# m4rch1n0/vqvae

Measured on AMD Instinct MI355X. Metric: latents/sec through geodesic kNN+APSP+K-medoids, higher is better.
Workload: dtype f64-exact(u32 fixed point)

## Files before the change

### include/geo_hip.h

```cpp
#ifndef GEO_HIP_H
#define GEO_HIP_H

#include <stddef.h>
#include <stdint.h>

#ifdef __cplusplus
extern "C" {
#endif

#define GEO_OK 0
#define GEO_E_ARG (-1)
#define GEO_E_WORKSPACE (-2)
#define GEO_E_HIP (-3)
#define GEO_E_NOCONV (-4)

int geo_version(void);
const char *geo_last_error(void);

int geo_set_option(const char *name, int32_t value);

size_t geo_sssp_workspace_bytes(int32_t n, int64_t nnz, int32_t n_sources);

int geo_sssp_multi(const int32_t *indptr, const int32_t *indices, const float *weights,
                   int32_t n, int64_t nnz, const int32_t *sources, int32_t n_sources,
// ... 129 lines not shown
                          const int32_t *src, const int32_t *dst, int64_t n_edges, int32_t batch_size,
                          float *len_out, void *ws, size_t ws_bytes, void *stream);
size_t geo_jvp_edges_part_workspace_bytes(const geo_decoder_desc *dec, int64_t n_nodes, int64_t n_edges, int64_t build_edges,
                                          int32_t batch_size);
int geo_decoder_jvp_edges_part(const geo_decoder_desc *dec, const float *z, int64_t n_nodes,
                               const int32_t *src, const int32_t *dst, int64_t n_edges, int64_t build_edges, int32_t batch_size,
                               float *len_out, void *ws, size_t ws_bytes, void *stream);

#define GEO_JVP_FRONT_VALU 0
#define GEO_JVP_FRONT_MFMA 1
#define GEO_JVP_MID_PIPE 0
#define GEO_JVP_MID_PIPE_DEDUP 1
#define GEO_JVP_MID_ALL 2
#define GEO_JVP_MID_ALL_TANGENT 3
#define GEO_JVP_MID_CHUNK 4
#define GEO_JVP_BACK_MFMA 0
#define GEO_JVP_BACK_PER_NODE 1
#define GEO_JVP_BACK_DEDUP 2
#define GEO_JVP_BACK_VALU 3
#define GEO_JVP_PLAN_FRONT(p) ((p) & 3)
#define GEO_JVP_PLAN_DMAX(p) (16 << (((p) >> 2) & 3))
#define GEO_JVP_PLAN_MID(p) (((p) >> 4) & 15)
#define GEO_JVP_PLAN_BACK(p) (((p) >> 8) & 15)
#define GEO_JVP_PER_NODE 0x1000
#define GEO_JVP_NODE_JACOBIAN 0x2000
#define GEO_JVP_DEDUP 0x4000
#define GEO_JVP_FRONT_ONCE 0x8000
#define GEO_JVP_PLAN_PASSES(p) ((p) >> 16)
int geo_jvp_plan(const geo_decoder_desc *dec, int64_t n_nodes, int64_t n_edges, int32_t batch_size, int32_t graph_edges,
                 size_t ws_bytes);
int geo_jvp_plan_part(const geo_decoder_desc *dec, int64_t n_nodes, int64_t n_edges, int64_t build_edges, int32_t batch_size,
                      int32_t graph_edges, size_t ws_bytes);
int geo_jvp_head_stream(const geo_decoder_desc *dec, int64_t n_nodes, int64_t n_edges, int32_t batch_size, int32_t graph_edges);

int geo_decoder_jvp_pairs(const geo_decoder_desc *dec, const float *z_start, const float *z_end,
                          int64_t n_edges, int32_t batch_size, float *len_out,
                          void *ws, size_t ws_bytes, void *stream);


typedef struct geo_vanilla_decoder_desc {
    int32_t latent_dim;
    int32_t c1, c2;
    int32_t out_channels;
    int32_t out_size;
    const float *At;
    const float *c;
    const float *w2p;
    const float *scale2;
    const float *shift2;
    const float *w3p;
    const float *b3;
} geo_vanilla_decoder_desc;

size_t geo_vanilla_jvp_workspace_bytes(const geo_vanilla_decoder_desc *dec, int64_t n_edges);
size_t geo_vanilla_jvp_edges_workspace_bytes(const geo_vanilla_decoder_desc *dec, int64_t n_nodes, int64_t n_edges);
int geo_vanilla_jvp_pairs(const geo_vanilla_decoder_desc *dec, const float *z_start, const float *z_end, int64_t n_edges,
                          int32_t batch_size, float *len_out, void *ws, size_t ws_bytes, void *stream);
int geo_vanilla_jvp_edges(const geo_vanilla_decoder_desc *dec, const float *z, int64_t n_nodes, const int32_t *src,
                          const int32_t *dst, int64_t n_edges, int32_t batch_size, float *len_out, void *ws, size_t ws_bytes,
                          void *stream);

size_t geo_vanilla_decode_workspace_bytes(const geo_vanilla_decoder_desc *dec, int64_t n);
int geo_vanilla_decode(const geo_vanilla_decoder_desc *dec, const float *z, const int32_t *index, int64_t n, float *logits_out,
                       void *ws, size_t ws_bytes, void *stream);

typedef struct geo_spatial_image_decoder_desc {
// ... 145 lines not shown
```

### vqvae_amd/_lib.py

```python
import ctypes
import os

import torch

_HERE = os.path.dirname(os.path.abspath(__file__))
LIB_PATH = os.path.join(_HERE, "libgeo_hip.so")

c_p = ctypes.c_void_p
i32, i64, sz = ctypes.c_int32, ctypes.c_int64, ctypes.c_size_t


class DecoderDesc(ctypes.Structure):
    _fields_ = ([(n, i32) for n in ("latent_dim", "c0", "c1", "c2", "out_channels", "out_size", "norm",
                                    "bn_train", "groups1", "groups2")]
                + [("eps", ctypes.c_float)]
                + [(n, c_p) for n in ("w_in", "b_in", "w1", "b1", "g1", "be1", "rm1", "rv1",
                                      "w2", "b2", "g2", "be2", "rm2", "rv2", "w3", "b3")]
                + [("update_running", i32), ("momentum", ctypes.c_float)])


class VanillaDecoderDesc(ctypes.Structure):
    _fields_ = ([(n, i32) for n in ("latent_dim", "c1", "c2", "out_channels", "out_size")]
                + [(n, c_p) for n in ("At", "c", "w2p", "scale2", "shift2", "w3p", "b3")])

# ... 45 lines not shown
    "geo_cell_costs_workspace_bytes": (sz, [i32, i64, i32, i32]),
    "geo_cell_costs_min_workspace_bytes": (sz, [i32, i64, i32, i32]),
    "geo_cell_costs": (ctypes.c_int, [c_p, c_p, c_p, i32, i64, c_p, c_p, c_p, i32, i32, i32, c_p, c_p, sz, c_p, c_p]),
    "geo_kpp_resident_max_nodes": (i32, []),
    "geo_kpp_chain": (ctypes.c_int, [c_p, c_p, c_p, i32, c_p, c_p, c_p, c_p, c_p, i32, i32, i32, i32, i32, c_p, sz, c_p, c_p]),
    "geo_knn_workspace_bytes": (sz, [i64, i32]),
    "geo_knn_topk": (ctypes.c_int, [c_p, i64, i32, i32, i32, i64, i64, c_p, c_p, c_p, sz, c_p]),
    "geo_knn_query_workspace_bytes": (sz, [i64, i64, i32]),
    "geo_knn_query_min_workspace_bytes": (sz, [i64, i32]),
    "geo_knn_query": (ctypes.c_int, [c_p, i64, c_p, i64, i32, i32, i32, c_p, c_p, c_p, sz, c_p]),
    "geo_knn_last_path": (ctypes.c_int, []),
    "geo_knn_thresholds": (ctypes.c_int, [c_p, i64, i32, i32, i32, i64, i64, i32, c_p, c_p, sz, c_p]),
    "geo_nearest_foreign_workspace_bytes": (sz, [i64, i32]),
    "geo_nearest_foreign": (ctypes.c_int, [c_p, i64, i32, i32, c_p, c_p, i64, c_p, c_p, c_p, sz, c_p]),
    "geo_bridge_components_workspace_bytes": (sz, [i64, i32, i32]),
    "geo_bridge_components": (ctypes.c_int, [c_p, i64, i32, i32, c_p, i32, c_p, c_p, c_p, c_p, sz, c_p]),
    "geo_csr_insert_workspace_bytes": (sz, [i32, i64]),
    "geo_csr_insert_count": (ctypes.c_int, [c_p, c_p, i32, c_p, c_p, c_p, i64, c_p, c_p, c_p, sz, c_p]),
    "geo_csr_insert_fill": (ctypes.c_int, [c_p, c_p, c_p, i32, i64, c_p, c_p, c_p, c_p, sz, c_p]),
    "geo_symmetrize_workspace_bytes": (sz, [i32, i32]),
    "geo_symmetrize_count": (ctypes.c_int, [c_p, c_p, i32, i32, i32, c_p, c_p, c_p, sz, c_p]),
    "geo_symmetrize_fill": (ctypes.c_int, [c_p, c_p, i32, i32, i32, c_p, c_p, c_p, c_p, sz, c_p]),
    "geo_upper_edges_count": (ctypes.c_int, [c_p, c_p, i32, c_p, c_p, c_p, sz, c_p]),
    "geo_upper_edges_fill": (ctypes.c_int, [c_p, c_p, i32, c_p, c_p, c_p, c_p, c_p]),
    "geo_cc_workspace_bytes": (sz, [i32]),
    "geo_connected_components": (ctypes.c_int, [c_p, c_p, i32, c_p, c_p, c_p, sz, c_p]),
    "geo_csr_compact_workspace_bytes": (sz, [i32]),
    "geo_csr_compact_count": (ctypes.c_int, [c_p, c_p, c_p, i32, c_p, i32, c_p, c_p, c_p, c_p, c_p, sz, c_p]),
    "geo_csr_compact_fill": (ctypes.c_int, [c_p, c_p, c_p, i32, c_p, i32, c_p, c_p, c_p, c_p, c_p]),
    "geo_jvp_workspace_bytes": (sz, [ctypes.POINTER(DecoderDesc), i64, i32]),
    "geo_jvp_edges_workspace_bytes": (sz, [ctypes.POINTER(DecoderDesc), i64, i64, i32]),
    "geo_jvp_plan": (ctypes.c_int, [ctypes.POINTER(DecoderDesc), i64, i64, i32, i32, sz]),
    "geo_jvp_head_stream": (ctypes.c_int, [ctypes.POINTER(DecoderDesc), i64, i64, i32, i32]),
    "geo_decoder_jvp_edges": (ctypes.c_int, [ctypes.POINTER(DecoderDesc), c_p, i64, c_p, c_p, i64, i32, c_p, c_p, sz, c_p]),
    "geo_jvp_edges_part_workspace_bytes": (sz, [ctypes.POINTER(DecoderDesc), i64, i64, i64, i32]),
    "geo_jvp_plan_part": (ctypes.c_int, [ctypes.POINTER(DecoderDesc), i64, i64, i64, i32, i32, sz]),
    "geo_decoder_jvp_edges_part": (ctypes.c_int, [ctypes.POINTER(DecoderDesc), c_p, i64, c_p, c_p, i64, i64, i32, c_p, c_p, sz,
                                                  c_p]),
    "geo_decoder_jvp_pairs": (ctypes.c_int, [ctypes.POINTER(DecoderDesc), c_p, c_p, i64, i32, c_p, c_p, sz, c_p]),
    "geo_vanilla_jvp_workspace_bytes": (sz, [ctypes.POINTER(VanillaDecoderDesc), i64]),
    "geo_vanilla_jvp_edges_workspace_bytes": (sz, [ctypes.POINTER(VanillaDecoderDesc), i64, i64]),
    "geo_vanilla_jvp_pairs": (ctypes.c_int, [ctypes.POINTER(VanillaDecoderDesc), c_p, c_p, i64, i32, c_p, c_p, sz, c_p]),
    "geo_vanilla_jvp_edges": (ctypes.c_int, [ctypes.POINTER(VanillaDecoderDesc), c_p, i64, c_p, c_p, i64, i32, c_p, c_p, sz, c_p]),
    "geo_vanilla_decode_workspace_bytes": (sz, [ctypes.POINTER(VanillaDecoderDesc), i64]),
    "geo_vanilla_decode": (ctypes.c_int, [ctypes.POINTER(VanillaDecoderDesc), c_p, c_p, i64, c_p, c_p, sz, c_p]),
    "geo_spatial_decode_workspace_bytes": (sz, [ctypes.POINTER(SpatialImageDecoderDesc), i64]),
    "geo_spatial_decode": (ctypes.c_int, [ctypes.POINTER(SpatialImageDecoderDesc), c_p, c_p, c_p, i64, c_p, c_p, sz, c_p]),
    "geo_image_encode_workspace_bytes": (sz, [ctypes.POINTER(ImageEncoderDesc), i64]),
    "geo_image_encode": (ctypes.c_int, [ctypes.POINTER(ImageEncoderDesc), c_p, i64, c_p, c_p, c_p, sz, c_p]),
    "geo_lpips_alex_workspace_bytes": (sz, [i64]),
    "geo_lpips_alex": (ctypes.c_int, [ctypes.POINTER(LPIPSAlexDesc), c_p, c_p, i64, c_p, c_p, c_p, sz, c_p]),
    "geo_gather_edge_weights":(ctypes.c_int, [c_p, c_p, i64, c_p, c_p]),
    "geo_prior_sample_workspace_bytes": (sz, [ctypes.POINTER(PriorDesc), i32, i32]),
    "geo_prior_sample": (ctypes.c_int, [ctypes.POINTER(PriorDesc), c_p, i32, i32, c_p, c_p, ctypes.c_float, i32, c_p, c_p, i32,
                                        c_p, sz, c_p]),
    "geo_kmeans_workspace_bytes": (sz, [i64, i32, i32, i32, i32]),
    "geo_kmeans_assign": (ctypes.c_int, [c_p, i64, i32, c_p, i32, c_p, c_p, c_p, c_p, sz, c_p]),
    "geo_kmeans_pp": (ctypes.c_int, [c_p, i64, i32, i32, i32, i32, c_p, c_p, c_p, c_p, c_p, sz, c_p]),
    "geo_kmeans_lloyd": (ctypes.c_int, [c_p, i64, i32, i32, i32, c_p, i32, ctypes.c_double, c_p, c_p, c_p, c_p, c_p, c_p, c_p,
                                        sz, c_p]),
    "geo_image_pair_moments": (ctypes.c_int, [c_p, c_p, i64, i64, c_p, c_p]),
    "geo_cluster_label_scores": (ctypes.c_int, [c_p, c_p, i64, i32, i32, i32, c_p, c_p, c_p, c_p, c_p, c_p]),
    "geo_feature_workspace_bytes": (sz, [i64, i32]),
    "geo_feature_colstats": (ctypes.c_int, [c_p, i64, i32, i64, c_p, c_p, c_p, c_p, sz, c_p]),
    "geo_feature_gram": (ctypes.c_int, [c_p, i64, i32, i64, c_p, c_p, c_p, c_p, sz, c_p]),
    "geo_feature_project": (ctypes.c_int, [c_p, i64, i32, i64, c_p, c_p, c_p, i32, c_p, c_p]),
# ... 57 lines not shown
```

### vqvae_amd/csrc/common.hip

```cpp
#include "geo_common.h"

#include <cstdlib>
#include <cstring>

namespace geo {

namespace {
struct OptionName { const char *name, *env; int Options::*field; };
const OptionName kOptionNames[] = {
    {"sssp_sb", "GEO_SSSP_SB", &Options::sssp_sb},
    {"sssp_act", "GEO_SSSP_ACT", &Options::sssp_act},
    {"sssp_sparse_div", "GEO_SSSP_SPARSE_DIV", &Options::sssp_sparse_div},
    {"sssp_map_div", "GEO_SSSP_MAP_DIV", &Options::sssp_map_div},
    {"sssp_group", "GEO_SSSP_GROUP", &Options::sssp_group},
    {"sssp_grouped_cap", "GEO_SSSP_GROUPED_CAP", &Options::sssp_grouped_cap},
    {"sssp_trace", "GEO_SSSP_TRACE", &Options::sssp_trace},
    {"sssp_u32", "GEO_SSSP_U32", &Options::sssp_u32},
    {"sssp_push", "GEO_SSSP_PUSH", &Options::sssp_push},
    {"sssp_order", "GEO_SSSP_ORDER", &Options::sssp_order},
    {"sssp_delta", "GEO_SSSP_DELTA", &Options::sssp_delta},
    {"sssp_push_blocks", "GEO_SSSP_PUSH_BLOCKS", &Options::sssp_push_blocks},
    {"knn_filter", "GEO_KNN_FILTER", &Options::knn_filter},
    {"kpp_grid", "GEO_KPP_GRID", &Options::kpp_grid},
    {"kpp_profile", "GEO_KPP_PROFILE", &Options::kpp_profile},
    {"jvp_mid", "GEO_JVP_MID", &Options::jvp_mid},
    {"jvp_back_valu", "GEO_JVP_BACK_VALU", &Options::jvp_back_valu},
    {"jvp_front_valu", "GEO_JVP_FRONT_VALU", &Options::jvp_front_valu},
    {"jvp_per_node", "GEO_JVP_PER_NODE", &Options::jvp_per_node},
    {"jvp_node_jacobian", "GEO_JVP_NODE_JACOBIAN", &Options::jvp_node_jacobian},
    {"jvp_start_dedup", "GEO_JVP_START_DEDUP", &Options::jvp_start_dedup},
    {"jvp_front_once", "GEO_JVP_FRONT_ONCE", &Options::jvp_front_once},
    {"jvp_head_stream", "GEO_JVP_HEAD_STREAM", &Options::jvp_head_stream},
};
Options from_environment() {
    Options o;
    for (const OptionName &e : kOptionNames) {
        const char *v = getenv(e.env);
        if (!v) continue;
        if (e.field == &Options::jvp_mid) o.jvp_mid = v[0] == 'c' ? 2 : (v[0] == 'a' ? 3 : atoi(v));
        else o.*(e.field) = atoi(v);
    }
    return o;
}
}

Options &options() {
    static Options o = from_environment();
    return o;
}

static thread_local char g_err[512] = "";

void set_error(const char *fmt, ...) {
    va_list ap;
    va_start(ap, fmt);
    vsnprintf(g_err, sizeof(g_err), fmt, ap);
    va_end(ap);
}

constexpr int SCAN_THREADS = 256;
constexpr int SCAN_ITEMS = 8;
constexpr int SCAN_TILE = SCAN_THREADS * SCAN_ITEMS;

__global__ __launch_bounds__(SCAN_THREADS) void scan_tiles_kernel(const int32_t *__restrict__ in,
                                                                 int32_t *__restrict__ out,
// ... 67 lines not shown
        set_error("exclusive_scan: workspace too small");
        return GEO_E_WORKSPACE;
    }
    scan_tiles_kernel<<<dim3((unsigned)t), dim3(SCAN_THREADS), 0, s>>>(in, out, sums, n);
    GEO_LAUNCH_CHECK();
    if (t == 1) {
        scan_single_total_kernel<<<1, 64, 0, s>>>(out, sums, n);
        GEO_LAUNCH_CHECK();
        return GEO_OK;
    }
    int rc = scan_rec(sums, offs, t, ar, s);
    if (rc != GEO_OK) return rc;
    scan_add_kernel<<<dim3((unsigned)t), dim3(SCAN_THREADS), 0, s>>>(out, offs, n, t);
    GEO_LAUNCH_CHECK();
    return GEO_OK;
}

int exclusive_scan_i32(const int32_t *in, int32_t *out, int64_t n, void *tmp, size_t tmp_bytes,
                       int64_t *total_host, hipStream_t stream) {
    Arena ar(tmp, tmp_bytes);
    int rc = scan_rec(in, out, n, ar, stream);
    if (rc != GEO_OK) return rc;
    if (total_host) {
        int32_t tot = 0;
        GEO_HIP_CHECK(hipMemcpyAsync(&tot, out + n, sizeof(int32_t), hipMemcpyDeviceToHost, stream));
        GEO_HIP_CHECK(hipStreamSynchronize(stream));
        *total_host = tot;
    }
    return GEO_OK;
}

}

extern "C" int geo_version(void) { return 114; }
extern "C" const char *geo_last_error(void) { return geo::g_err; }

extern "C" int geo_set_option(const char *name, int32_t value) {
    if (name)
        for (const geo::OptionName &e : geo::kOptionNames)
            if (strcmp(name, e.name) == 0) {
                geo::options().*(e.field) = value;
                return GEO_OK;
            }
    geo::set_error("geo_set_option: unknown option '%s'", name ? name : "(null)");
    return GEO_E_ARG;
}
```

### vqvae_amd/csrc/geo_common.h

```cpp
#pragma once
#include <hip/hip_runtime.h>

#include <cstdarg>
#include <cstdint>
#include <cstdio>

#include "geo_hip.h"

namespace geo {

void set_error(const char *fmt, ...);

#define GEO_HIP_CHECK(expr)                                                                      \
    do {                                                                                         \
        hipError_t _e = (expr);                                                                  \
        if (_e != hipSuccess) {                                                                  \
            geo::set_error("%s failed: %s (%s:%d)", #expr, hipGetErrorString(_e), __FILE__, __LINE__); \
            return GEO_E_HIP;                                                                    \
        }                                                                                        \
    } while (0)

#define GEO_REQUIRE(cond, ...)              \
    do {                                    \
        if (!(cond)) {                      \
            geo::set_error(__VA_ARGS__);    \
            return GEO_E_ARG;               \
        }                                   \
    } while (0)

#define GEO_LAUNCH_CHECK() GEO_HIP_CHECK(hipGetLastError())

struct Options {
    int sssp_sb = -1, sssp_act = 1, sssp_sparse_div = -1, sssp_map_div = -1, sssp_group = 1, sssp_grouped_cap = 256,
        sssp_trace = 0, sssp_u32 = 1, sssp_push = 1 ,
        sssp_delta = 8 , sssp_order = 0 , sssp_push_blocks = 64, knn_filter = 1, kpp_grid = 256, kpp_profile = 0, jvp_mid = 0 ,
        jvp_back_valu = 0, jvp_front_valu = 0, jvp_per_node = 1 ,
        jvp_node_jacobian = 1 ,
        jvp_start_dedup = 1 ,
        jvp_front_once = 1 ,
        jvp_head_stream = 1 ;
};
Options &options();

static inline size_t align_up(size_t x, size_t a = 256) { return (x + a - 1) / a * a; }

struct Arena {
    char *base;
    size_t size, off;
    Arena(void *p, size_t n) : base(static_cast<char *>(p)), size(n), off(0) {}
    template <typename T>
    T *take(size_t count) {
        size_t bytes = align_up(count * sizeof(T));
        if (off + bytes > size) return nullptr;
        T *r = reinterpret_cast<T *>(base + off);
        off += bytes;
        return r;
    }
};

static inline int64_t shrink_pass(int64_t items) { return items > 64 ? items - items / 8 : items - 1; }

static inline size_t pass_bytes(const size_t *per_item, int nb, int64_t items) {
    size_t bytes = 0;
    for (int b = 0; b < nb; ++b) bytes += align_up((size_t)items * per_item[b] * 4);
    return bytes;
}

static inline size_t pass_query_bytes(const size_t *per_item, int nb, int64_t cap, int64_t n) {
    return pass_bytes(per_item, nb, n < 1 ? 1 : (n < cap ? n : cap));
}

static inline int plan_passes(const char *who, const size_t *per_item, int nb, int64_t cap, int64_t n, void *ws, size_t ws_bytes,
                              int64_t *items, float **bufs) {
// ... 31 lines not shown
```

### vqvae_amd/csrc/jvp.hip

```cpp
#include "geo_common.h"

#include <cmath>
#include <cstdlib>
#include <type_traits>
#include <vector>

namespace {

constexpr int TS = 32;
constexpr int NC = 128;
constexpr int MAX_BLOCKS = 4;
constexpr int FRONT_MAX_N1 = 1024;
constexpr int BACK_TS = 8;

typedef float f32x16 __attribute__((ext_vector_type(16)));
typedef __bf16 bf16x8 __attribute__((ext_vector_type(8)));
typedef unsigned short u16x8 __attribute__((ext_vector_type(8)));

struct Shape {
    int d, c0, c1, c2, co, s_out, pad3, p_out;
    int n1, n2;
    int opix_per_chunk, n_chunks;
};

// ... 1302 lines not shown
        if (cnt_g > batch) cnt_g = batch;
#pragma unroll
        for (int hh = 0; hh < 2; ++hh) {
            if (hh == 1 && !live1) break;
            const int tile = hh ? tile1 : tile0;
            const size_t tbase = (size_t)tile * TS;
            const int n_valid = (int)cnt_g - (tile - group * tiles_per_group) * TS;
            Bn2Sums sums;
#pragma unroll
            for (int lc = 0; lc < NL; ++lc) {
                const int ch = wg == 0 ? MidGeom::chunk_of(0, lc) : MidGeom::chunk_of(1, lc);
                const int op = lo == 0 ? MidGeom::opix(ch, 0) : MidGeom::opix(ch, 1);
#pragma unroll
                for (int q = 0; q < 16; ++q) {
                    const int row = (q & 3) + 8 * (q >> 2) + 4 * h;
                    const float x = pre2[(size_t)row_map[tbase + row] * n2 + (size_t)op * c2 + co];
                    bn2_add(sums, x, hh ? acct[lc][q] : accp[lc][q], row < n_valid);
                }
            }
            bn2_store(sums, partial2, tile, wg * 2 + (wq >> 1), co, lane);
        }
    }
    };
    if (TT) {
        run((int)blockIdx.x);
    } else {
        for (int item = 0; 2 * item * TS < ncomp; ++item) {
            if (item > 0) { __builtin_amdgcn_s_setprio(0); __syncthreads(); }
            run(item);
        }
    }
}

__global__ __launch_bounds__(256) void slot_valid_kernel(int64_t e_base, int64_t n_edges, int batch, int tiles_per_group,
                                                        int64_t n_slots, int32_t *__restrict__ slot_valid) {
    for (int64_t i = (int64_t)blockIdx.x * blockDim.x + threadIdx.x; i < n_slots; i += (int64_t)gridDim.x * blockDim.x) {
        const int64_t per_group = (int64_t)tiles_per_group * TS;
        const int64_t g = i / per_group, within = i % per_group;
        const int64_t e = e_base + (g >> 1) * batch + within;
        slot_valid[i] = (within < batch && e < n_edges) ? 1 : 0;
    }
}

__global__ __launch_bounds__(256) void slot_node_kernel(const int32_t *__restrict__ src, const int32_t *__restrict__ dst,
                                                       int64_t e_base, int64_t n_edges, int batch, int tiles_per_group,
                                                       int64_t n_slots, int32_t *__restrict__ slot_node) {
    for (int64_t i = (int64_t)blockIdx.x * blockDim.x + threadIdx.x; i < n_slots; i += (int64_t)gridDim.x * blockDim.x) {
        const int64_t per_group = (int64_t)tiles_per_group * TS;
        const int64_t g = i / per_group, within = i % per_group;
        const int64_t e = e_base + (g >> 1) * batch + within;
        slot_node[i] = (within < batch && e < n_edges) ? ((g & 1) ? dst[e] : src[e]) : 0;
    }
}

__global__ __launch_bounds__(256) void back_kernel(const float *__restrict__ pre2, const float *__restrict__ tpre2,
                                                  const NormConst *__restrict__ consts2, int consts_per_group,
                                                  int slots_per_group, int c2, int co_n, int s_out, int pad3,
                                                  const float *__restrict__ W3p, const float *__restrict__ b3,
                                                  float *__restrict__ norms) {
    extern __shared__ __attribute__((aligned(16))) float smem[];
    const int n2 = 16 * c2;
    const int p_out = co_n * s_out * s_out;
    const int ldc = c2 + 4;
    const int lds_n2 = 16 * ldc;
    float *a2 = smem;
    float *ta2 = a2 + (size_t)BACK_TS * lds_n2;
// ... 522 lines not shown
    p->chunks_per_pass = cpp;
    const Shape &s = p->sh;
    const size_t slots = p->pass_slots(), tiles = slots / TS, groups = (size_t)cpp * 2;
    size_t b = 0;
    b += geo::align_up((size_t)s.d * s.n1 * 4) + geo::align_up((size_t)s.n1 * 4);
    b += geo::align_up((size_t)s.n_chunks * MAX_BLOCKS * s.c1 * NC * 4);
    b += geo::align_up((size_t)s.n_chunks * MAX_BLOCKS * s.c1 * NC * 2 * 3);
    b += geo::align_up((size_t)16 * s.co * s.c2 * 4);
    b += geo::align_up((size_t)16 * s.c2 * 192 * 3 * 2);
    b += 2 * geo::align_up(slots * s.n1 * 4) + 2 * geo::align_up(slots * s.n2 * 4);
    b += geo::align_up(tiles * s.n1 * 4 * 8) + geo::align_up(tiles * s.n2 * 4 * 8);
    b += geo::align_up((groups + 1) * s.c1 * sizeof(NormConst)) + geo::align_up((groups + 1) * s.c2 * sizeof(NormConst));
    b += geo::align_up((groups + 1) * (size_t)(s.c1 > s.c2 ? s.c1 : s.c2) * sizeof(float2));
    b += geo::align_up(slots * 4) * 2;
    if (dc->norm == 2) b += 2 * geo::align_up(slots * 32 * sizeof(float4));
    p->bytes = b + 4096;
    return true;
}

enum { BACK_NODE_PRIMAL = 15 };

struct Route {
    int status = GEO_OK;
    char error[192] = "";
    Plan pl = {};
    int64_t run_edges = 0, passes = 0;
    bool batch_stats = false, track = false, group_norm = false;
    int front = GEO_JVP_FRONT_VALU, dmax = 16;
    int mid = GEO_JVP_MID_CHUNK, back = GEO_JVP_BACK_VALU;
    int back_nt = 0;
    int parts2 = 16;
    bool per_node = false, node_jacobian = false, dedup = false, front_once = false;
    bool head_stream = false;
    size_t back_lds = 0;
    size_t jac_np = 0, jac_extra_bytes = 0;
    size_t bytes = 0;
};

bool route_error(Route *r, int status, const char *fmt, ...) {
    va_list ap;
    va_start(ap, fmt);
    vsnprintf(r->error, sizeof(r->error), fmt, ap);
    va_end(ap);
    r->status = status;
    return false;
}

bool make_route(const geo_decoder_desc *dc, const geo::Options &o, bool graph_edges, int64_t n_nodes, int64_t n_edges,
                int64_t build_edges, int batch, const size_t *ws_bytes, Route *r) {
    *r = Route{};
    if (!dc) return route_error(r, GEO_E_ARG, "geo_decoder_jvp: null pointer");
    if (batch <= 0) return route_error(r, GEO_E_ARG, "geo_decoder_jvp: batch_size must be positive");
    if (build_edges < n_edges)
        return route_error(r, GEO_E_ARG, "geo_decoder_jvp: build_edges %lld < n_edges %lld", (long long)build_edges,
                           (long long)n_edges);
    Plan base;
    if (n_edges < 0 || n_nodes < 0 || !make_plan(dc, n_edges, batch, &base))
        return route_error(r, GEO_E_ARG, "geo_decoder_jvp: unsupported decoder (out_size %d, c2=%d must divide %d)", dc->out_size,
                           dc->c2, NC);
    const Shape &s = base.sh;

    r->batch_stats = dc->norm == 1 && dc->bn_train;
    r->track = r->batch_stats && dc->update_running && dc->rm1 && dc->rv1 && dc->rm2 && dc->rv2;
    r->group_norm = dc->norm == 2;
    r->dmax = s.d <= 16 ? 16 : (s.d <= 32 ? 32 : 64);
    r->front = s.d > 16 && s.n1 % 32 == 0 && o.jvp_front_valu == 0 ? GEO_JVP_FRONT_MFMA : GEO_JVP_FRONT_VALU;
// ... 11 lines not shown
    if (per_node_kernels && n_nodes > 0 && n_edges > 0 && s.d <= 16 && o.jvp_node_jacobian != 0 &&
        (o.jvp_node_jacobian != 1 || 4 * build_edges >= 3 * n_nodes * s.d) && n_pseudo < (int64_t)1 << 31 &&
        make_plan(dc, n_pseudo, batch, &jpl) && node_slots <= jpl.pass_slots()) {
        r->jac_np = (size_t)r->back_nt * 32;
        r->jac_extra_bytes = 2 * geo::align_up((size_t)n_pseudo * 4) + geo::align_up((size_t)n_nodes * s.d * r->jac_np * 4);
        jac_bytes = r->jac_extra_bytes + jpl.bytes + node_bytes(s, n_nodes);
    }
    r->bytes = jac_bytes > per_edge_end_bytes ? jac_bytes : per_edge_end_bytes;
    const size_t ws = ws_bytes ? *ws_bytes : r->bytes;
    r->node_jacobian = jac_bytes && ws >= jac_bytes;
    r->pl = r->node_jacobian ? jpl : base;
    r->run_edges = r->node_jacobian ? n_pseudo : n_edges;
    const int64_t chunks = (r->run_edges + batch - 1) / batch;
    r->passes = (chunks + r->pl.chunks_per_pass - 1) / r->pl.chunks_per_pass;
    const size_t run_ws = ws - (r->node_jacobian ? r->jac_extra_bytes : 0);
    r->per_node = per_node_kernels && node_slots && node_slots <= r->pl.pass_slots() &&
                  run_ws >= r->pl.bytes + node_bytes(s, n_nodes);
    const size_t slots = r->pl.pass_slots(), tiles = slots / TS, groups = (size_t)r->pl.chunks_per_pass * 2;
    r->dedup = r->batch_stats && graph_edges && mid_pipe && back_mfma && o.jvp_start_dedup != 0 &&
               (2 * slots + groups) * 4 <= tiles * s.n1 * 4 * 8 && (size_t)r->back_nt * 32 <= (size_t)s.n1;
    r->front_once = r->dedup && r->front == GEO_JVP_FRONT_VALU && o.jvp_front_once != 0 && s.n1 == FRONT_EDGE_N1 &&
                    tiles * s.c1 * 4 * 8 + (2 * slots + groups) * 4 <= tiles * s.n1 * 4 * 8 &&
                    (size_t)base.slots_per_group * s.n1 * 4 < ((size_t)1 << 31);

    r->mid = r->per_node ? GEO_JVP_MID_ALL_TANGENT
           : mid_pipe    ? (r->dedup ? GEO_JVP_MID_PIPE_DEDUP : GEO_JVP_MID_PIPE)
           : mid_all     ? GEO_JVP_MID_ALL
                         : GEO_JVP_MID_CHUNK;
    r->parts2 = mid_pipe && !r->per_node ? 4 : (mid_all ? 1 : 16);
    r->back = r->dedup ? GEO_JVP_BACK_DEDUP : r->per_node ? GEO_JVP_BACK_PER_NODE : back_mfma ? GEO_JVP_BACK_MFMA : GEO_JVP_BACK_VALU;
    r->head_stream = back_mfma && r->back_nt == 1 && !r->group_norm && (r->back == GEO_JVP_BACK_DEDUP || r->back == GEO_JVP_BACK_MFMA) &&
                     o.jvp_head_stream != 0 &&
                     (!r->dedup || (size_t)base.slots_per_group * s.n2 * 4 < ((size_t)1 << 31));
    r->back_lds = ((size_t)2 * BACK_TS * 16 * (s.c2 + 4) + (size_t)16 * s.co * (s.c2 + 4) + (size_t)BACK_TS * s.p_out) * 4;

    if (!(s.d >= 1 && s.d <= 64)) return route_error(r, GEO_E_ARG, "geo_decoder_jvp: latent_dim %d not in [1,64]", s.d);
    if (!(s.c1 == 128 || s.c1 == 64 || s.c1 == 32))
        return route_error(r, GEO_E_ARG, "geo_decoder_jvp: dec_channels[1]=%d not in {32,64,128}", s.c1);
    if (!(dc->norm >= 0 && dc->norm <= 2)) return route_error(r, GEO_E_ARG, "geo_decoder_jvp: unknown norm code %d", dc->norm);
    if (s.c2 % 16 != 0) return route_error(r, GEO_E_ARG, "geo_decoder_jvp: dec_channels[2]=%d must be a multiple of 16", s.c2);
    if (r->back_lds > 160 * 1024)
        return route_error(r, GEO_E_ARG, "geo_decoder_jvp: decoder too wide for the back kernel (%zu B LDS)", r->back_lds);
    if (run_ws < r->pl.bytes) return route_error(r, GEO_E_WORKSPACE, "geo_decoder_jvp: workspace %zu < %zu", run_ws, r->pl.bytes);
    if (r->group_norm && !(dc->groups1 == 32 && dc->groups2 == 32 && s.c2 == 64 && back_mfma && mid_all))
        return route_error(r, GEO_E_ARG,
                           "geo_decoder_jvp: GroupNorm needs 32 groups per layer and dec_channels[2] == 64 (got %d/%d groups, c2=%d)",
                           dc->groups1, dc->groups2, s.c2);
    return true;
}

int encode_route(const Route &r) {
    const int64_t passes = r.passes < 0x7fff ? r.passes : 0x7fff;
    return r.front | (r.dmax == 16 ? 0 : (r.dmax == 32 ? 1 : 2)) << 2 | r.mid << 4 | r.back << 8 |
           (r.per_node ? GEO_JVP_PER_NODE : 0) | (r.node_jacobian ? GEO_JVP_NODE_JACOBIAN : 0) | (r.dedup ? GEO_JVP_DEDUP : 0) |
           (r.front_once ? GEO_JVP_FRONT_ONCE : 0) | (int)passes << 16;
}

struct Buffers {
    float *M01, *b01, *B2p, *W3p, *pre1, *tpre1, *pre2, *tpre2, *norms;
    unsigned short *B3, *W3b;
    double *part1, *part2; NormConst *k1, *k2;
    float2 *stats;
    int32_t *slot_valid;
    float4 *gs1, *gs2;
    float *pre2_node, *sg_node;
    int32_t *row_map, *rep, *n_compact;
// ... 80 lines not shown
            slot_node_kernel<<<geo::grid_for(p.slots(), 256), 256, 0, stream>>>(p.src, p.dst, p.e_base, p.n_edges, p.batch,
                                                                                p.tiles_per_group, p.slots(), b.slot_valid);
            prim_row = b.slot_valid;
        }
        group_stats_kernel<<<geo::grid_for(p.slots() * 32, 256), 256, 0, stream>>>(
            l1 ? b.pre1 : p.back_pre2, l1 ? b.tpre1 : b.tpre2, p.slots(), npx, C, 32, dc->eps, l1 ? b.gs1 : b.gs2, prim_row);
        GEO_LAUNCH_CHECK();
    }
    return GEO_OK;
}

int launch_mid(const Route &r, const geo_decoder_desc *dc, const Pass &p, const Buffers &b, hipStream_t stream) {
    const Shape &s = r.pl.sh;
    if (p.mid == GEO_JVP_MID_PIPE || p.mid == GEO_JVP_MID_PIPE_DEDUP) {
        const bool dedup = p.mid == GEO_JVP_MID_PIPE_DEDUP;
        const int64_t chunks = p.groups() / 2;
        if (dedup && !r.front_once)
            if (const int rc = launch_start_runs(p, b, stream)) return rc;
        int n_cu = 0;
        if (const int rc = cu_count(&n_cu)) return rc;
        const int64_t pipe_tiles = dedup ? p.tiles / 2 : p.tiles;
        const unsigned grid = (unsigned)std::min<int64_t>(pipe_tiles, n_cu);
        pick_bool(dedup, [&](auto end_only) {
            mid_pipe_kernel<decltype(end_only)::value><<<grid, 512, 0, stream>>>(
                b.pre1, b.tpre1, b.k1, p.stat, p.tiles_per_group, (int)pipe_tiles, s.c2, b.B3, dc->b2, p.mid_pre2, b.tpre2, b.part2,
                p.stat, p.e_base, p.n_edges, p.batch);
        });
        GEO_LAUNCH_CHECK();
        if (dedup) {
            mid_start_kernel<false><<<dim3(1, (unsigned)chunks), 512, 0, stream>>>(
                b.pre1, b.tpre1, b.k1, p.tiles_per_group, b.B3, dc->b2, p.mid_pre2, b.tpre2, b.part2, b.row_map, b.rep, b.n_compact,
                p.e_base, p.n_edges, p.batch);
            GEO_LAUNCH_CHECK();
            pick_bool(r.front_once, [&](auto once) {
                mid_start_kernel<true, decltype(once)::value>
                    <<<dim3((unsigned)((p.tiles_per_group + 1) / 2), (unsigned)chunks), 512, 0, stream>>>(
                        b.pre1, b.tpre1, b.k1, p.tiles_per_group, b.B3, dc->b2, p.mid_pre2, b.tpre2, b.part2, b.row_map, b.rep,
                        b.n_compact, p.e_base, p.n_edges, p.batch);
            });
            GEO_LAUNCH_CHECK();
        }
    } else if (p.mid == GEO_JVP_MID_ALL || p.mid == GEO_JVP_MID_ALL_TANGENT) {
        pick_int<128, 64, 32>(s.c1, [&](auto c1) {
            pick_bool(r.group_norm, [&](auto gn) {
                pick_bool(p.mid == GEO_JVP_MID_ALL_TANGENT, [&](auto tangent_only) {
                    mid_all_kernel<decltype(c1)::value, decltype(gn)::value, decltype(tangent_only)::value>
                        <<<(unsigned)p.tiles, 512, 0, stream>>>(b.pre1, b.tpre1, b.k1, p.stat, p.tiles_per_group, s.c2, b.B3, dc->b2,
                                                                p.mid_pre2, b.tpre2, b.part2, p.stat, b.slot_valid, b.gs1, p.e_base,
                                                                p.n_edges, p.batch);
                });
            });
        });
        GEO_LAUNCH_CHECK();
    } else {
        pick_int<128, 64, 32>(s.c1, [&](auto c1) {
            mid_bf16_kernel<decltype(c1)::value><<<dim3((unsigned)p.tiles, (unsigned)s.n_chunks), 256, 0, stream>>>(
                b.pre1, b.tpre1, b.k1, p.stat, p.tiles_per_group, b.tab, s.opix_per_chunk, s.c2, b.B3, dc->b2, p.mid_pre2, b.tpre2,
                b.part2, p.stat, b.slot_valid);
        });
        GEO_LAUNCH_CHECK();
    }
    return GEO_OK;
}

int launch_back(const Route &r, const geo_decoder_desc *dc, const Pass &p, const Buffers &b, hipStream_t stream) {
    const Shape &s = r.pl.sh;
    if (p.back == GEO_JVP_BACK_VALU) {
        back_kernel<<<(unsigned)(p.slots() / BACK_TS), 256, r.back_lds, stream>>>(
            p.back_pre2, b.tpre2, b.k2, p.stat, p.tiles_per_group * TS, s.c2, s.co, s.s_out, s.pad3, b.W3p, dc->b3, b.norms);
        GEO_LAUNCH_CHECK();
        return GEO_OK;
    }
// ... 162 lines not shown
    }
    if (r.node_jacobian) {
        const int64_t teams = (n_edges * 16 + 255) / 256;
        GEO_REQUIRE(teams < ((int64_t)1 << 31), "geo_decoder_jvp_edges: too many edges for one launch (%lld)", (long long)n_edges);
        jacobian_lengths_kernel<<<(unsigned)teams, 256, 0, stream>>>(z, src, dst, n_edges, s.d, s.p_out, (int)r.jac_np, b.jac, len_out);
        GEO_LAUNCH_CHECK();
    }
    return GEO_OK;
}

int decoder_jvp(const geo_decoder_desc *dc, const geo::Options &opt, bool graph_edges, const float *z, int64_t n_nodes,
                const int32_t *src, const int32_t *dst, const float *z_start, const float *z_end, int64_t n_edges,
                int64_t build_edges, int32_t batch, float *len_out, void *ws, size_t ws_bytes, void *stream) {
    GEO_REQUIRE(dc && len_out && ws, "geo_decoder_jvp: null pointer");
    GEO_REQUIRE(batch > 0, "geo_decoder_jvp: batch_size must be positive");
    if (n_edges == 0) return GEO_OK;
    Route r;
    if (!make_route(dc, opt, graph_edges, n_nodes, n_edges, build_edges, batch, &ws_bytes, &r)) {
        geo::set_error("%s", r.error);
        return r.status;
    }
    return run_jvp(dc, r, z, n_nodes, src, dst, z_start, z_end, n_edges, len_out, ws, ws_bytes, static_cast<hipStream_t>(stream));
}

}

#ifdef GEO_MID_PROF
extern "C" int geo_debug_mid_prof(unsigned long long *out, int reset) {
    if (reset) { unsigned long long z[16] = {0}; return (int)hipMemcpyToSymbol(HIP_SYMBOL(g_mid_prof), z, sizeof(z)); }
    return (int)hipMemcpyFromSymbol(out, HIP_SYMBOL(g_mid_prof), sizeof(unsigned long long) * 16);
}
#endif

extern "C" size_t geo_jvp_workspace_bytes(const geo_decoder_desc *dec, int64_t n_edges, int32_t batch_size) {
    const geo::Options opt = geo::options();
    Route r;
    make_route(dec, opt, false, 0, n_edges, n_edges, batch_size, nullptr, &r);
    return r.bytes;
}

extern "C" size_t geo_jvp_edges_part_workspace_bytes(const geo_decoder_desc *dec, int64_t n_nodes, int64_t n_edges,
                                                     int64_t build_edges, int32_t batch_size) {
    const geo::Options opt = geo::options();
    Route r;
    make_route(dec, opt, true, n_nodes, n_edges, build_edges, batch_size, nullptr, &r);
    return r.bytes;
}

extern "C" size_t geo_jvp_edges_workspace_bytes(const geo_decoder_desc *dec, int64_t n_nodes, int64_t n_edges,
                                                int32_t batch_size) {
    return geo_jvp_edges_part_workspace_bytes(dec, n_nodes, n_edges, n_edges, batch_size);
}

extern "C" int geo_jvp_plan_part(const geo_decoder_desc *dec, int64_t n_nodes, int64_t n_edges, int64_t build_edges,
                                 int32_t batch_size, int32_t graph_edges, size_t ws_bytes) {
    const geo::Options opt = geo::options();
    Route r;
    if (!make_route(dec, opt, graph_edges != 0, graph_edges ? n_nodes : 0, n_edges, build_edges, batch_size,
                    ws_bytes ? &ws_bytes : nullptr, &r)) {
        geo::set_error("%s", r.error);
        return r.status;
    }
    return encode_route(r);
}

extern "C" int geo_jvp_plan(const geo_decoder_desc *dec, int64_t n_nodes, int64_t n_edges, int32_t batch_size,
                            int32_t graph_edges, size_t ws_bytes) {
    return geo_jvp_plan_part(dec, n_nodes, n_edges, n_edges, batch_size, graph_edges, ws_bytes);
}

extern "C" int geo_jvp_head_stream(const geo_decoder_desc *dec, int64_t n_nodes, int64_t n_edges, int32_t batch_size,
                                   int32_t graph_edges) {
    const geo::Options opt = geo::options();
    Route r;
    if (!make_route(dec, opt, graph_edges != 0, graph_edges ? n_nodes : 0, n_edges, n_edges, batch_size, nullptr, &r)) {
        geo::set_error("%s", r.error);
        return r.status;
    }
    return r.head_stream ? 1 : 0;
}

extern "C" int geo_decoder_jvp_edges_part(const geo_decoder_desc *dec, const float *z, int64_t n_nodes, const int32_t *src,
                                          const int32_t *dst, int64_t n_edges, int64_t build_edges, int32_t batch_size,
                                          float *len_out, void *ws, size_t ws_bytes, void *stream) {
    GEO_REQUIRE(build_edges >= n_edges, "geo_decoder_jvp_edges_part: build_edges %lld < n_edges %lld", (long long)build_edges,
                (long long)n_edges);
    GEO_REQUIRE(n_edges == 0 || (z && src && dst && n_nodes > 0), "geo_decoder_jvp_edges: null pointer");
    const geo::Options opt = geo::options();
    return decoder_jvp(dec, opt, true, z, n_nodes, src, dst, nullptr, nullptr, n_edges, build_edges, batch_size, len_out, ws,
                       ws_bytes, stream);
}

extern "C" int geo_decoder_jvp_edges(const geo_decoder_desc *dec, const float *z, int64_t n_nodes, const int32_t *src,
                                     const int32_t *dst, int64_t n_edges, int32_t batch_size, float *len_out, void *ws,
                                     size_t ws_bytes, void *stream) {
    return geo_decoder_jvp_edges_part(dec, z, n_nodes, src, dst, n_edges, n_edges, batch_size, len_out, ws, ws_bytes, stream);
}

extern "C" int geo_decoder_jvp_pairs(const geo_decoder_desc *dec, const float *z_start, const float *z_end,
                                     int64_t n_edges, int32_t batch_size, float *len_out, void *ws, size_t ws_bytes,
                                     void *stream) {
    GEO_REQUIRE(n_edges == 0 || (z_start && z_end), "geo_decoder_jvp_pairs: null pointer");
    const geo::Options opt = geo::options();
    return decoder_jvp(dec, opt, false, nullptr, 0, nullptr, nullptr, z_start, z_end, n_edges, n_edges, batch_size, len_out, ws,
                       ws_bytes, stream);
}
```

Measured before the change: 2.525 million.

## Add persistent software-pipelined mid-start kernel overlapping fetch, staging, MFMA and epilogue

Adds a persistent kernel, launched with at most one block per CU, that loops over (chunk, tile-pair) items. It double-buffers the normalised start activations in LDS and prefetches the next item's row map, representative offsets and inputs while the current item's MFMA products and epilogue run, with the two wave groups staggered. The aim is to hide global-memory latency and remove per-block launch and ramp-up cost of the original grid-per-item mid_start_kernel. It is enabled by default when front_once is set, adds a query entry point and an optional profiling hook, and in exchange raises register and LDS pressure and adds scheduling complexity.

```diff
diff --git a/include/geo_hip.h b/include/geo_hip.h
--- a/include/geo_hip.h
+++ b/include/geo_hip.h
@@ -185,6 +185,7 @@
 int geo_jvp_plan_part(const geo_decoder_desc *dec, int64_t n_nodes, int64_t n_edges, int64_t build_edges, int32_t batch_size,
                       int32_t graph_edges, size_t ws_bytes);
 int geo_jvp_head_stream(const geo_decoder_desc *dec, int64_t n_nodes, int64_t n_edges, int32_t batch_size, int32_t graph_edges);
+int geo_jvp_start_pipe(const geo_decoder_desc *dec, int64_t n_nodes, int64_t n_edges, int32_t batch_size, int32_t graph_edges);
 
 int geo_decoder_jvp_pairs(const geo_decoder_desc *dec, const float *z_start, const float *z_end,
                           int64_t n_edges, int32_t batch_size, float *len_out,
diff --git a/vqvae_amd/_lib.py b/vqvae_amd/_lib.py
--- a/vqvae_amd/_lib.py
+++ b/vqvae_amd/_lib.py
@@ -101,6 +101,7 @@
     "geo_jvp_edges_workspace_bytes": (sz, [ctypes.POINTER(DecoderDesc), i64, i64, i32]),
     "geo_jvp_plan": (ctypes.c_int, [ctypes.POINTER(DecoderDesc), i64, i64, i32, i32, sz]),
     "geo_jvp_head_stream": (ctypes.c_int, [ctypes.POINTER(DecoderDesc), i64, i64, i32, i32]),
+    "geo_jvp_start_pipe": (ctypes.c_int, [ctypes.POINTER(DecoderDesc), i64, i64, i32, i32]),
     "geo_decoder_jvp_edges": (ctypes.c_int, [ctypes.POINTER(DecoderDesc), c_p, i64, c_p, c_p, i64, i32, c_p, c_p, sz, c_p]),
     "geo_jvp_edges_part_workspace_bytes": (sz, [ctypes.POINTER(DecoderDesc), i64, i64, i64, i32]),
     "geo_jvp_plan_part": (ctypes.c_int, [ctypes.POINTER(DecoderDesc), i64, i64, i64, i32, i32, sz]),
diff --git a/vqvae_amd/csrc/common.hip b/vqvae_amd/csrc/common.hip
--- a/vqvae_amd/csrc/common.hip
+++ b/vqvae_amd/csrc/common.hip
@@ -31,6 +31,7 @@
     {"jvp_start_dedup", "GEO_JVP_START_DEDUP", &Options::jvp_start_dedup},
     {"jvp_front_once", "GEO_JVP_FRONT_ONCE", &Options::jvp_front_once},
     {"jvp_head_stream", "GEO_JVP_HEAD_STREAM", &Options::jvp_head_stream},
+    {"jvp_start_pipe", "GEO_JVP_START_PIPE", &Options::jvp_start_pipe},
 };
 Options from_environment() {
     Options o;
@@ -164,7 +165,7 @@
 
 }
 
-extern "C" int geo_version(void) { return 114; }
+extern "C" int geo_version(void) { return 115; }
 extern "C" const char *geo_last_error(void) { return geo::g_err; }
 
 extern "C" int geo_set_option(const char *name, int32_t value) {
diff --git a/vqvae_amd/csrc/geo_common.h b/vqvae_amd/csrc/geo_common.h
--- a/vqvae_amd/csrc/geo_common.h
+++ b/vqvae_amd/csrc/geo_common.h
@@ -38,7 +38,8 @@
         jvp_node_jacobian = 1 ,
         jvp_start_dedup = 1 ,
         jvp_front_once = 1 ,
-        jvp_head_stream = 1 ;
+        jvp_head_stream = 1 ,
+        jvp_start_pipe = 1 ;
 };
 Options &options();
 
diff --git a/vqvae_amd/csrc/jvp.hip b/vqvae_amd/csrc/jvp.hip
--- a/vqvae_amd/csrc/jvp.hip
+++ b/vqvae_amd/csrc/jvp.hip
@@ -1358,6 +1358,263 @@
     }
 }
 
+#ifdef GEO_START_PROF
+__device__ unsigned long long g_start_prof[2][8];
+#endif
+__global__ __launch_bounds__(512, 2) void mid_start_pipe_kernel(const float *__restrict__ pre1, const float *__restrict__ tpre1,
+                                                               const NormConst *__restrict__ consts1, int tiles_per_group,
+                                                               int pairs_per_group, int n_items,
+                                                               const unsigned short *__restrict__ B3, const float *__restrict__ pre2,
+                                                               float *__restrict__ tpre2, double *__restrict__ partial2,
+                                                               const int32_t *__restrict__ row_map, const int32_t *__restrict__ rep,
+                                                               int64_t e_base, int64_t n_edges, int batch) {
+    constexpr int C1 = 128, LDK = C1 + 8, KS = C1 / 16, NL = 4, c2 = 64, n1 = 4 * C1, n2 = 16 * c2;
+    typedef float f32x2 __attribute__((ext_vector_type(2)));
+    __shared__ __attribute__((aligned(16))) unsigned short A3[2][3][2][TS][LDK];
+    const int lane = threadIdx.x & 63, wave = __builtin_amdgcn_readfirstlane((int)(threadIdx.x >> 6));
+    const int wq = wave & 3, wg = wave >> 2;
+    const int r = lane & 31, h = lane >> 5;
+    const int k0p = 2 * lane;
+    const int lo = wq >> 1, co = (wq & 1) * 32 + r;
+    const unsigned v_out = (unsigned)(4 * h * n2 + co) * 4u;
+    const int my_items = (n_items - (int)blockIdx.x + (int)gridDim.x - 1) / (int)gridDim.x;
+    if (my_items <= 0) return;
+    const int group_slots = tiles_per_group * TS;
+
+    f32x16 accp[NL], acct[NL];
+    auto zero_acc = [&]() {
+#pragma unroll
+        for (int lc = 0; lc < NL; ++lc)
+#pragma unroll
+            for (int i = 0; i < 16; ++i) { accp[lc][i] = 0.f; acct[lc][i] = 0.f; }
+    };
+    zero_acc();
+    auto split_item = [&](int item, int &chunk, int &lt0) {
+        chunk = item / pairs_per_group;
+        lt0 = 2 * (item - chunk * pairs_per_group);
+    };
+    int st_chunk, st_lt0;
+    NormConst kA, kB;
+    f32x2 rx[2][2], rt[2][2];
+    unsigned v_heads = 0;
+    auto load_consts = [&]() {
+        const NormConst *kp = consts1 + (size_t)(2 * st_chunk) * C1 + k0p;
+        kA = kp[0];
+        kB = kp[1];
+    };
+    const int lk_hh = lane < 8 ? lane >> 2 : ((lane - 8) >> 3) & 1;
+    const int lk_row = lane < 8 ? 4 * wave + (lane & 3) : 8 * wq + ((lane - 8) & 7);
+    auto lookup_map = [&](int chunk, int lt0) {
+        const int lt = lk_hh && lt0 + 1 < tiles_per_group ? lt0 + 1 : lt0;
+        return row_map[(size_t)2 * chunk * group_slots + lt * TS + lk_row];
+    };
+    auto lookup_rep = [&](int chunk, int rm) { return (unsigned)(rep[rm] - 2 * chunk * group_slots) * (n1 * 4u); };
+    const unsigned v_pair = (unsigned)k0p * 4u;
+    auto fetch = [&](int px, auto full_tag, auto unit_tag) {
+        constexpr bool FULL = decltype(full_tag)::value;
+        constexpr int U = decltype(unit_tag)::value;
+        const size_t g0 = (size_t)2 * st_chunk * group_slots;
+        const __amdgpu_buffer_rsrc_t x_src = __builtin_amdgcn_make_buffer_rsrc(const_cast<float *>(pre1 + g0 * n1), 0, group_slots * n1 * 4, 0x00020000);
+        const __amdgpu_buffer_rsrc_t t_src = __builtin_amdgcn_make_buffer_rsrc(const_cast<float *>(tpre1 + (g0 + group_slots) * n1), 0, group_slots * n1 * 4, 0x00020000);
+        const int row0 = (FULL ? 8 * wq : 4 * wave) + 2 * U;
+        const int px_off = MidGeom::pix(px) * C1 * 4;
+#pragma unroll
+        for (int hh = 0; hh < 2; ++hh) {
+            const int lt = hh && st_lt0 + 1 < tiles_per_group ? st_lt0 + 1 : st_lt0;
+            const int toff = (lt * TS + row0) * n1 * 4 + px_off;
+#pragma unroll
+            for (int i = 0; i < 2; ++i) {
+                const int xoff = __builtin_amdgcn_readlane((int)v_heads, (FULL ? 8 + hh * 8 : hh * 4) + 2 * U + i);
+                rx[hh][i] = __builtin_bit_cast(f32x2, __builtin_amdgcn_raw_buffer_load_b64(x_src, v_pair, xoff + px_off, 0));
+                rt[hh][i] = __builtin_bit_cast(f32x2, __builtin_amdgcn_raw_buffer_load_b64(t_src, v_pair, toff + i * n1 * 4, 0));
+            }
+        }
+        __builtin_amdgcn_sched_group_barrier(0x020, 8, 0);
+    };
+    auto stage = [&](int buf, auto full_tag, auto unit_tag) {
+        constexpr bool FULL = decltype(full_tag)::value;
+        constexpr int U = decltype(unit_tag)::value;
+        const int row0 = (FULL ? 8 * wq : 4 * wave) + 2 * U;
+        unsigned w_idx = (unsigned)((buf * 3 * 2 * TS + row0) * LDK + k0p);
+        asm volatile("" : "+v"(w_idx));
+        unsigned short *w = &A3[0][0][0][0][0] + w_idx;
+#pragma unroll
+        for (int hh = 0; hh < 2; ++hh)
+#pragma unroll
+            for (int i = 0; i < 2; ++i) {
+                float a0, t0, a1, t1;
+                norm_relu(kA, rx[hh][i].x, rt[hh][i].x, &a0, &t0);
+                norm_relu(kB, rx[hh][i].y, rt[hh][i].y, &a1, &t1);
+                unsigned wt[3];
+                split3_pair(t0, t1, wt[0], wt[1], wt[2]);
+#pragma unroll
+                for (int part = 0; part < 3; ++part)
+                    *reinterpret_cast<unsigned *>(w + ((part * 2 + hh) * TS + i) * LDK) = wt[part];
+            }
+    };
+    std::true_type FULL;
+    std::false_type HALF;
+    std::integral_constant<int, 0> U0;
+    std::integral_constant<int, 1> U1;
+    std::integral_constant<int, 2> U2;
+    std::integral_constant<int, 3> U3;
+
+    bf16x8 ring[3][3];
+    const unsigned b_lane = (unsigned)(h * 3 * NC * 8 + (wq * 32 + r) * 8) * 2u;
+    const __amdgpu_buffer_rsrc_t b_rsrc = __builtin_amdgcn_make_buffer_rsrc(
+        const_cast<unsigned short *>(B3), 0, (int)((size_t)8 * MAX_BLOCKS * C1 * NC * 3 * 2), 0x00020000);
+    auto ring_init = [&]() {
+        const int cb0 = wg == 0 ? MidGeom::prod_cb(0, MidGeom::pix(0), 0) : MidGeom::prod_cb(1, MidGeom::pix(0), 0);
+        const int cb1 = wg == 0 ? MidGeom::prod_cb(0, MidGeom::pix(0), 1) : MidGeom::prod_cb(1, MidGeom::pix(0), 1);
+#pragma unroll
+        for (int part = 0; part < 3; ++part) {
+            ring[0][part] = __builtin_bit_cast(bf16x8, __builtin_amdgcn_raw_buffer_load_b128(b_rsrc, b_lane, (cb0 * KS * 2 * 3 + part) * NC * 8 * 2, 0));
+            ring[1][part] = __builtin_bit_cast(bf16x8, __builtin_amdgcn_raw_buffer_load_b128(b_rsrc, b_lane, (cb1 * KS * 2 * 3 + part) * NC * 8 * 2, 0));
+        }
+    };
+    auto epilogue = [&](int chunk, int lt0) {
+#ifdef GEO_START_PROF
+        const unsigned long long t_e = __builtin_amdgcn_s_memtime();
+#endif
+        const int group = 2 * chunk;
+        int64_t cnt_g = n_edges - (e_base + (int64_t)chunk * batch);
+        if (cnt_g > batch) cnt_g = batch;
+        const int g0 = group * group_slots;
+        const __amdgpu_buffer_rsrc_t x_src = __builtin_amdgcn_make_buffer_rsrc(const_cast<float *>(pre2 + (size_t)g0 * n2), 0, group_slots * n2 * 4, 0x00020000);
+#pragma unroll
+        for (int hh = 0; hh < 2; ++hh) {
+            if (hh == 1 && !(lt0 + 1 < tiles_per_group)) break;
+            const int lt = lt0 + hh, tile = group * tiles_per_group + lt;
+            const int n_valid = (int)cnt_g - lt * TS;
+            const __amdgpu_buffer_rsrc_t t_dst = __builtin_amdgcn_make_buffer_rsrc(tpre2 + (size_t)tile * TS * n2, 0, TS * n2 * 4, 0x00020000);
+            unsigned vrow[16];
+#pragma unroll
+            for (int q = 0; q < 16; ++q)
+                vrow[q] = (unsigned)(row_map[(size_t)tile * TS + (q & 3) + 8 * (q >> 2) + 4 * h] - g0) * (n2 * 4u) + (unsigned)co * 4u;
+            float xs[2][16];
+            auto gather = [&](int lc) {
+                const int ch = wg == 0 ? MidGeom::chunk_of(0, lc) : MidGeom::chunk_of(1, lc);
+                const int op = lo == 0 ? MidGeom::opix(ch, 0) : MidGeom::opix(ch, 1);
+#pragma unroll
+                for (int q = 0; q < 16; ++q)
+                    xs[lc & 1][q] = __uint_as_float(__builtin_amdgcn_raw_buffer_load_b32(x_src, vrow[q], op * c2 * 4, 0));
+            };
+            gather(0);
+            Bn2Sums sums;
+#pragma unroll
+            for (int lc = 0; lc < NL; ++lc) {
+                const int ch = wg == 0 ? MidGeom::chunk_of(0, lc) : MidGeom::chunk_of(1, lc);
+                const int op = lo == 0 ? MidGeom::opix(ch, 0) : MidGeom::opix(ch, 1);
+                if (lc + 1 < NL) gather(lc + 1);
+#pragma unroll
+                for (int q = 0; q < 16; ++q) {
+                    const float t = hh ? acct[lc][q] : accp[lc][q];
+                    const int soff = (((q & 3) + 8 * (q >> 2)) * n2 + op * c2) * 4;
+                    __builtin_amdgcn_raw_buffer_store_b32(__float_as_uint(t), t_dst, v_out, soff, 0);
+                    bn2_add(sums, xs[lc & 1][q], t, 4 * h < n_valid - ((q & 3) + 8 * (q >> 2)));
+                }
+            }
+            bn2_store(sums, partial2, tile, wg * 2 + (wq >> 1), co, lane);
+        }
+        zero_acc();
+#ifdef GEO_START_PROF
+        if (lane == 0 && wq == 0) atomicAdd(&g_start_prof[wg][6], __builtin_amdgcn_s_memtime() - t_e);
+#endif
+    };
+
+    const unsigned short *a3 = &A3[0][0][0][0][0];
+    const unsigned a_lane = (unsigned)(r * LDK + h * 8);
+    constexpr unsigned A_BUF = 3u * 2u * TS * LDK;
+#define GEO_PIPE_PIXEL(WGV, IPV)                                                                                       \
+    mid_products<C1, false, WGV, IPV>(a3, a_lane + ((IPV) & 1) * A_BUF, b_rsrc, b_lane, accp, acct, ring)
+#define GEO_PIPE_SEP() __builtin_amdgcn_sched_barrier(0)
+#define GEO_STAGE_HALF(BUF, PX)                                                                                         \
+    { stage(BUF, HALF, U0); fetch(PX, HALF, U1); GEO_PIPE_SEP(); stage(BUF, HALF, U1); }
+#define GEO_STAGE_FULL(BUF, PX)                                                                                         \
+    { stage(BUF, FULL, U0); fetch(PX, FULL, U1); GEO_PIPE_SEP(); stage(BUF, FULL, U1); fetch(PX, FULL, U2); GEO_PIPE_SEP();       \
+      stage(BUF, FULL, U2); fetch(PX, FULL, U3); GEO_PIPE_SEP(); stage(BUF, FULL, U3); }
+
+    int item = blockIdx.x, cur_chunk, cur_lt0;
+    split_item(item, cur_chunk, cur_lt0);
+    st_chunk = cur_chunk; st_lt0 = cur_lt0;
+    v_heads = lookup_rep(st_chunk, lookup_map(st_chunk, st_lt0));
+    load_consts();
+    fetch(0, HALF, U0);
+    ring_init();
+    GEO_STAGE_HALF(0, 0);
+    if (wg == 0) fetch(1, FULL, U0);
+    else fetch(2, HALF, U0);
+    if (wg == 0) __builtin_amdgcn_s_setprio(1);
+    lds_barrier();
+#ifdef GEO_START_PROF
+    unsigned long long pb_prev = __builtin_amdgcn_s_memtime();
+#define GEO_PB(slot)                                                                                                   \
+    { const unsigned long long t_a = __builtin_amdgcn_s_memtime();                                                      \
+      lds_barrier();                                                                                                    \
+      const unsigned long long t_b = __builtin_amdgcn_s_memtime();                                                      \
+      if (lane == 0 && wq == 0) { atomicAdd(&g_start_prof[wg][1 + slot], t_a - pb_prev); atomicAdd(&g_start_prof[wg][5], t_b - t_a); \
+                                  if (slot == 3) atomicAdd(&g_start_prof[wg][7], 1ull); }                               \
+      pb_prev = t_b; }
+#else
+#define GEO_PB(slot) lds_barrier();
+#endif
+    if (wg == 0) {
+        for (int it = 0; it < my_items; ++it) {
+            const bool has_next = it + 1 < my_items;
+            const int next = has_next ? item + (int)gridDim.x : item;
+            int nx_chunk, nx_lt0;
+            split_item(next, nx_chunk, nx_lt0);
+            GEO_PIPE_PIXEL(0, 0); GEO_PIPE_SEP();
+            GEO_STAGE_FULL(1, 1); fetch(2, HALF, U0); GEO_PB(0);
+            GEO_PIPE_PIXEL(0, 1); GEO_PIPE_SEP(); GEO_STAGE_HALF(0, 2); fetch(3, HALF, U0); GEO_PB(1);
+            const int v_map = lookup_map(nx_chunk, nx_lt0); GEO_PIPE_SEP();
+            GEO_PIPE_PIXEL(0, 2); GEO_PIPE_SEP(); GEO_STAGE_HALF(1, 3); GEO_PB(2);
+            const unsigned v_off = lookup_rep(nx_chunk, v_map); GEO_PIPE_SEP();
+            GEO_PIPE_PIXEL(0, 3); GEO_PIPE_SEP();
+            epilogue(cur_chunk, cur_lt0);
+            GEO_PIPE_SEP();
+            if (has_next) {
+                st_chunk = nx_chunk; st_lt0 = nx_lt0;
+                v_heads = v_off; load_consts(); fetch(1, FULL, U0); ring_init();
+            }
+            GEO_PB(3);
+            item = next; cur_chunk = nx_chunk; cur_lt0 = nx_lt0;
+        }
+    } else {
+        int prev_chunk = cur_chunk, prev_lt0 = cur_lt0;
+        for (int it = 0; it < my_items; ++it) {
+            const bool has_next = it + 1 < my_items;
+            const int next = has_next ? item + (int)gridDim.x : item;
+            int nx_chunk, nx_lt0;
+            split_item(next, nx_chunk, nx_lt0);
+            if (it > 0) { epilogue(prev_chunk, prev_lt0); GEO_PIPE_SEP(); ring_init(); }
+            GEO_PIPE_PIXEL(1, 0); GEO_PB(0);
+            const int v_map = lookup_map(nx_chunk, nx_lt0);
+            GEO_STAGE_HALF(0, 2); fetch(3, HALF, U0); GEO_PIPE_SEP();
+            GEO_PIPE_PIXEL(1, 1); GEO_PB(1);
+            const unsigned v_off = lookup_rep(nx_chunk, v_map);
+            GEO_STAGE_HALF(1, 3);
+            if (has_next) {
+                st_chunk = nx_chunk; st_lt0 = nx_lt0;
+                v_heads = v_off; load_consts(); fetch(0, FULL, U0);
+            }
+            GEO_PIPE_SEP();
+            GEO_PIPE_PIXEL(1, 2); GEO_PB(2);
+            if (has_next) { GEO_STAGE_FULL(0, 0); fetch(2, HALF, U0); }
+            GEO_PIPE_SEP();
+            GEO_PIPE_PIXEL(1, 3); GEO_PB(3);
+            prev_chunk = cur_chunk; prev_lt0 = cur_lt0;
+            item = next; cur_chunk = nx_chunk; cur_lt0 = nx_lt0;
+        }
+        epilogue(prev_chunk, prev_lt0);
+    }
+#undef GEO_STAGE_FULL
+#undef GEO_STAGE_HALF
+#undef GEO_PIPE_SEP
+#undef GEO_PB
+#undef GEO_PIPE_PIXEL
+}
+
 __global__ __launch_bounds__(256) void slot_valid_kernel(int64_t e_base, int64_t n_edges, int batch, int tiles_per_group,
                                                         int64_t n_slots, int32_t *__restrict__ slot_valid) {
     for (int64_t i = (int64_t)blockIdx.x * blockDim.x + threadIdx.x; i < n_slots; i += (int64_t)gridDim.x * blockDim.x) {
@@ -1946,6 +2203,7 @@
     int parts2 = 16;
     bool per_node = false, node_jacobian = false, dedup = false, front_once = false;
     bool head_stream = false;
+    bool start_pipe = false;
     size_t back_lds = 0;
     size_t jac_np = 0, jac_extra_bytes = 0;
     size_t bytes = 0;
@@ -2023,6 +2281,7 @@
     r->head_stream = back_mfma && r->back_nt == 1 && !r->group_norm && (r->back == GEO_JVP_BACK_DEDUP || r->back == GEO_JVP_BACK_MFMA) &&
                      o.jvp_head_stream != 0 &&
                      (!r->dedup || (size_t)base.slots_per_group * s.n2 * 4 < ((size_t)1 << 31));
+    r->start_pipe = r->front_once && o.jvp_start_pipe != 0 && (size_t)base.slots_per_group * s.n2 * 4 < ((size_t)1 << 31);
     r->back_lds = ((size_t)2 * BACK_TS * 16 * (s.c2 + 4) + (size_t)16 * s.co * (s.c2 + 4) + (size_t)BACK_TS * s.p_out) * 4;
 
     if (!(s.d >= 1 && s.d <= 64)) return route_error(r, GEO_E_ARG, "geo_decoder_jvp: latent_dim %d not in [1,64]", s.d);
@@ -2169,12 +2428,19 @@
                 b.pre1, b.tpre1, b.k1, p.tiles_per_group, b.B3, dc->b2, p.mid_pre2, b.tpre2, b.part2, b.row_map, b.rep, b.n_compact,
                 p.e_base, p.n_edges, p.batch);
             GEO_LAUNCH_CHECK();
-            pick_bool(r.front_once, [&](auto once) {
-                mid_start_kernel<true, decltype(once)::value>
-                    <<<dim3((unsigned)((p.tiles_per_group + 1) / 2), (unsigned)chunks), 512, 0, stream>>>(
+            const int pairs = (p.tiles_per_group + 1) / 2;
+            if (r.start_pipe) {
+                const int64_t items = chunks * pairs;
+                mid_start_pipe_kernel<<<(unsigned)std::min<int64_t>(items, n_cu), 512, 0, stream>>>(
+                    b.pre1, b.tpre1, b.k1, p.tiles_per_group, pairs, (int)items, b.B3, p.mid_pre2, b.tpre2, b.part2, b.row_map, b.rep,
+                    p.e_base, p.n_edges, p.batch);
+            } else {
+                pick_bool(r.front_once, [&](auto once) {
+                    mid_start_kernel<true, decltype(once)::value><<<dim3((unsigned)pairs, (unsigned)chunks), 512, 0, stream>>>(
                         b.pre1, b.tpre1, b.k1, p.tiles_per_group, b.B3, dc->b2, p.mid_pre2, b.tpre2, b.part2, b.row_map, b.rep,
                         b.n_compact, p.e_base, p.n_edges, p.batch);
-            });
+                });
+            }
             GEO_LAUNCH_CHECK();
         }
     } else if (p.mid == GEO_JVP_MID_ALL || p.mid == GEO_JVP_MID_ALL_TANGENT) {
@@ -2403,6 +2669,13 @@
 }
 #endif
 
+#ifdef GEO_START_PROF
+extern "C" int geo_debug_start_prof(unsigned long long *out, int reset) {
+    if (reset) { unsigned long long z[16] = {0}; return (int)hipMemcpyToSymbol(HIP_SYMBOL(g_start_prof), z, sizeof(z)); }
+    return (int)hipMemcpyFromSymbol(out, HIP_SYMBOL(g_start_prof), sizeof(unsigned long long) * 16);
+}
+#endif
+
 extern "C" size_t geo_jvp_workspace_bytes(const geo_decoder_desc *dec, int64_t n_edges, int32_t batch_size) {
     const geo::Options opt = geo::options();
     Route r;
@@ -2449,6 +2722,17 @@
         return r.status;
     }
     return r.head_stream ? 1 : 0;
+}
+
+extern "C" int geo_jvp_start_pipe(const geo_decoder_desc *dec, int64_t n_nodes, int64_t n_edges, int32_t batch_size,
+                                  int32_t graph_edges) {
+    const geo::Options opt = geo::options();
+    Route r;
+    if (!make_route(dec, opt, graph_edges != 0, graph_edges ? n_nodes : 0, n_edges, n_edges, batch_size, nullptr, &r)) {
+        geo::set_error("%s", r.error);
+        return r.status;
+    }
+    return r.start_pipe ? 1 : 0;
 }
 
 extern "C" int geo_decoder_jvp_edges_part(const geo_decoder_desc *dec, const float *z, int64_t n_nodes, const int32_t *src,
```

New measurement: 2.539 million (median of 3 runs). Within noise of the previous version (+0.6%).
